# Gaius-Augustus/Augustus

Hardware: AMD Instinct MI355X
Metric: Mbp DNA decoded/sec (whole node), ab-initio human model (higher is better)
Workload: dtype f64; 1 GPU; synthetic uniform-random DNA, 100 contigs x 1000000 bp per GPU, --species=human ab initio (47 states, sample=0); pieces_in_flight_per_gpu=100, batches_in_flight_per_gpu=1

## Files before the change

augustus_amd/__init__.py:

```python
import ctypes
import sys
import os

_HERE = os.path.dirname(os.path.abspath(__file__))
LIB_PATH = os.environ.get("AUGX_LIB") or os.path.join(_HERE, "libaugx.so")

AUGX_E_ARG = -1
AUGX_E_NODEVICE = -3
AUGX_E_HIP = -4
AUGX_E_UNSUPPORTED = -5
AUGX_E_NOPATH = -6
AUGX_E_NOMEM = -7
AUGX_E_RANGE = -8


class AugxError(RuntimeError):
    def __init__(self, code, msg):
        super().__init__("augx error %d: %s" % (code, msg))
        self.code = code


class _Piece(ctypes.Structure):
    _fields_ = [("seq", ctypes.c_char_p), ("len", ctypes.c_int64), ("init_kind", ctypes.c_int32),
                ("term_kind", ctypes.c_int32)]
# ... 24 lines not shown
        L.augx_model_tables.restype = ctypes.c_void_p
        L.augx_model_tables.argtypes = [ctypes.c_void_p]
        L.augx_model_option.restype = ctypes.c_char_p
        L.augx_model_option.argtypes = [ctypes.c_void_p, ctypes.c_char_p]
        L.augx_model_destroy.argtypes = [ctypes.c_void_p]
        L.augx_device_count.restype = ctypes.c_int
        L.augx_partition_lpt.argtypes = [ctypes.c_void_p, ctypes.c_int, ctypes.c_int, ctypes.c_void_p]
        L.augx_decode_sharded.argtypes = [ctypes.c_void_p, ctypes.c_int, ctypes.c_void_p, ctypes.c_int, ctypes.c_void_p]
        L.augx_decoder_create.argtypes = [ctypes.c_void_p, ctypes.c_int, ctypes.POINTER(ctypes.c_void_p)]
        L.augx_decoder_destroy.argtypes = [ctypes.c_void_p]
        L.augx_decoder_set_share.argtypes = [ctypes.c_void_p, ctypes.c_int]
        L.augx_decoder_set_exact.argtypes = [ctypes.c_void_p, ctypes.c_int]
        L.augx_decoder_batch_capacity.restype = ctypes.c_int64
        L.augx_decoder_batch_capacity.argtypes = [ctypes.c_void_p]
        L.augx_batch_create.argtypes = [ctypes.c_void_p, ctypes.c_void_p, ctypes.c_int, ctypes.POINTER(ctypes.c_void_p)]
        L.augx_batch_decode.argtypes = [ctypes.c_void_p, ctypes.c_void_p]
        L.augx_batch_sync.argtypes = [ctypes.c_void_p]
        L.augx_batch_paths.argtypes = [ctypes.c_void_p, ctypes.c_void_p, ctypes.c_void_p]
        L.augx_batch_cells.argtypes = [ctypes.c_void_p, ctypes.c_void_p, ctypes.c_int, ctypes.c_void_p]
        L.augx_batch_prep.argtypes = [ctypes.c_void_p, ctypes.c_void_p, ctypes.c_int, ctypes.c_int, ctypes.c_int, ctypes.c_void_p, ctypes.c_int64,
                                      ctypes.POINTER(ctypes.c_int64)]
        L.augx_batch_kernel_ms.argtypes = [ctypes.c_void_p, ctypes.c_void_p, ctypes.POINTER(ctypes.c_float),
                                           ctypes.POINTER(ctypes.c_float), ctypes.POINTER(ctypes.c_float)]
        L.augx_batch_forward.argtypes = [ctypes.c_void_p, ctypes.c_void_p]
        L.augx_batch_forward_cells.argtypes = [ctypes.c_void_p, ctypes.c_void_p, ctypes.c_int, ctypes.c_void_p, ctypes.POINTER(ctypes.c_double)]
        L.augx_batch_destroy.argtypes = [ctypes.c_void_p]
        L.augx_rand_create.restype = ctypes.c_void_p
        L.augx_rand_create.argtypes = [ctypes.c_uint]
        L.augx_rand_next.argtypes = [ctypes.c_void_p]
        L.augx_rand_destroy.argtypes = [ctypes.c_void_p]
        L.augx_batch_sample.argtypes = [ctypes.c_void_p, ctypes.c_void_p, ctypes.c_int, ctypes.c_int, ctypes.c_void_p, ctypes.c_void_p]
        L.augx_decode_sampled.argtypes = [ctypes.c_void_p, ctypes.c_int, ctypes.c_void_p, ctypes.c_int, ctypes.c_int, ctypes.c_void_p,
                                          ctypes.c_void_p, ctypes.c_void_p]
        L.augx_format_gff_sampled.argtypes = [ctypes.c_void_p, ctypes.c_char_p, ctypes.c_char_p, ctypes.c_int64, ctypes.c_void_p, ctypes.c_int,
                                              ctypes.c_int, ctypes.c_void_p, ctypes.c_void_p, ctypes.c_int, ctypes.c_char_p, ctypes.c_int64,
                                              ctypes.POINTER(ctypes.c_int)]
        L.augx_path_free.argtypes = [ctypes.c_void_p]
        _lib = L
    return _lib


def _check(rc):
    if rc != 0:
        raise AugxError(rc, lib().augx_last_error().decode(errors="replace"))


# ... 65 lines not shown


class DecodedPiece:
    __slots__ = ("status", "ln_viterbi", "states")

    def __init__(self, status, lnv, states):
        self.status, self.ln_viterbi, self.states = status, lnv, states


class Batch:

    def __init__(self, decoder, seqs, init_kind=0, term_kind=0):
        L = lib()
        self.decoder = decoder
        self.n = len(seqs)
        self._keep = [s if isinstance(s, bytes) else s.encode() for s in seqs]
        self.lens = [len(s) for s in self._keep]
        P = (_Piece * self.n)()
        iks = init_kind if isinstance(init_kind, (list, tuple)) else [init_kind] * self.n
        tks = term_kind if isinstance(term_kind, (list, tuple)) else [term_kind] * self.n
        for i, s in enumerate(self._keep):
            P[i].seq, P[i].len, P[i].init_kind, P[i].term_kind = s, len(s), iks[i], tks[i]
        self._h = ctypes.c_void_p()
        _check(L.augx_batch_create(decoder._h, P, self.n, ctypes.byref(self._h)))
        decoder._batches.add(self._h.value)

    def decode(self, sync=True):
        _check(lib().augx_batch_decode(self.decoder._h, self._h))
        if sync:
            _check(lib().augx_batch_sync(self.decoder._h))

    def kernel_ms(self):
        a, b, c = ctypes.c_float(), ctypes.c_float(), ctypes.c_float()
        _check(lib().augx_batch_kernel_ms(self.decoder._h, self._h, ctypes.byref(a), ctypes.byref(b), ctypes.byref(c)))
        return {"prep_ms": a.value, "trellis_ms": b.value, "backtrace_ms": c.value}

    def paths(self):
        L = lib()
        out = (_Path * self.n)()
        _check(L.augx_batch_paths(self.decoder._h, self._h, out))
        res = []
        for i in range(self.n):
            st = [(out[i].states[k].begin, out[i].states[k].end, out[i].states[k].state, out[i].states[k].type)
                  for k in range(out[i].n_states)]
            res.append(DecodedPiece(out[i].status, out[i].ln_viterbi, st))
            L.augx_path_free(ctypes.byref(out[i]))
        return res

    def cells(self, piece):
        import numpy as np
        S = self.decoder.model.n_states
        V = np.empty((self.lens[piece], S), dtype=np.float64)
        _check(lib().augx_batch_cells(self.decoder._h, self._h, piece, V.ctypes.data_as(ctypes.c_void_p)))
        return V

    def prep(self, piece, which, plane=0):
        L = lib()
        return prep_fetch(lambda w, pl, out, cap, nb: L.augx_batch_prep(self.decoder._h, self._h, piece, w, pl, out, cap, nb), which, plane)

    def forward(self):
        _check(lib().augx_batch_forward(self.decoder._h, self._h))

    def forward_cells(self, piece):
        import numpy as np
        S = self.decoder.model.n_states
        F = np.empty((self.lens[piece], S), dtype=np.float64)
        lnp = ctypes.c_double()
        _check(lib().augx_batch_forward_cells(self.decoder._h, self._h, piece, F.ctypes.data_as(ctypes.c_void_p), ctypes.byref(lnp)))
        return F, lnp.value

    def sample(self, piece, n, rand):
        L = lib()
        out = (_Path * max(1, n))()
        _check(L.augx_batch_sample(self.decoder._h, self._h, piece, n, rand._h, out))
        res = []
        for i in range(n):
            if out[i].status != 0:
                raise AugxError(out[i].status, "sampling failed")
            res.append([(out[i].states[k].begin, out[i].states[k].end, out[i].states[k].state, out[i].states[k].type)
                        for k in range(out[i].n_states)])
            L.augx_path_free(ctypes.byref(out[i]))
# ... 83 lines not shown

def find_cuts(model, seqs, decode_fn, scout=-1):
    L = lib()
    L.augx_find_cuts.argtypes = [ctypes.c_void_p, ctypes.c_int, ctypes.POINTER(ctypes.c_char_p), ctypes.POINTER(ctypes.c_int64), DECODE_FN, ctypes.c_void_p,
                                 ctypes.c_int, ctypes.POINTER(ctypes.POINTER(_Cut)), ctypes.POINTER(ctypes.c_int), ctypes.POINTER(_CutStats)]
    L.augx_cuts_free.argtypes = [ctypes.POINTER(_Cut)]
    keep = [s.encode() if isinstance(s, str) else s for s in seqs]
    n = len(keep)
    c_seqs = (ctypes.c_char_p * n)(*keep)
    c_lens = (ctypes.c_int64 * n)(*[len(s) for s in keep])
    out = ctypes.POINTER(_Cut)()
    n_out = ctypes.c_int()
    st = _CutStats()
    _check(L.augx_find_cuts(model._h, n, c_seqs, c_lens, decode_fn, None, scout, ctypes.byref(out), ctypes.byref(n_out), ctypes.byref(st)))
    res = [(out[i].record, out[i].status, out[i].begin, out[i].end, out[i].init_kind, out[i].term_kind) for i in range(n_out.value)]
    L.augx_cuts_free(out)
    return res, {"scout_tiles": st.scout_tiles, "batches": st.batches, "windows_decoded": st.windows_decoded, "windows_used": st.windows_used}


def device_count():
    return lib().augx_device_count()


def partition_lpt(lens, n_bins):
    import numpy as np
    a = np.asarray(lens, dtype=np.int64)
    out = np.zeros(len(a), dtype=np.int32)
    _check(lib().augx_partition_lpt(a.ctypes.data_as(ctypes.c_void_p), len(a), n_bins, out.ctypes.data_as(ctypes.c_void_p)))
    return out.tolist()


def decode_sharded(decoders, seqs, init_kind=0, term_kind=0):
    L = lib()
    n = len(seqs)
    keep = [s if isinstance(s, bytes) else s.encode() for s in seqs]
    P = (_Piece * n)()
    iks = init_kind if isinstance(init_kind, (list, tuple)) else [init_kind] * n
    tks = term_kind if isinstance(term_kind, (list, tuple)) else [term_kind] * n
    for i, s in enumerate(keep):
        P[i].seq, P[i].len, P[i].init_kind, P[i].term_kind = s, len(s), iks[i], tks[i]
    D = (ctypes.c_void_p * len(decoders))(*[d._h for d in decoders])
    out = (_Path * n)()
    _check(L.augx_decode_sharded(D, len(decoders), P, n, out))
    res = []
    for i in range(n):
        st = [(out[i].states[k].begin, out[i].states[k].end, out[i].states[k].state, out[i].states[k].type)
# ... 54 lines not shown
```

augustus_amd/csrc/device/decoder.hip:

```cpp
#include <hip/hip_runtime.h>
#include <sys/mman.h>
#include <algorithm>
#include <map>
#include <array>
#include <cmath>
#include <unordered_map>
#include <cstdio>
#include <cstdlib>
#include <cstring>
#include <future>
#include <memory>
#include <mutex>
#include <set>
#include <string>
#include <system_error>
#include <thread>
#include <atomic>
#include <chrono>
#include <vector>
#include "kernels.h"
#include "dense.h"
#include "layout.h"
#include "launch.h"
#include "assmemo.h"
// ... 788 lines not shown
    keep(V.lnv, n); keep(V.status, n); keep(V.finalState, n); keep(V.pathCount, n);
    {
        std::vector<double> v;
        {
            std::lock_guard<std::mutex> lk(g_tss0Mu);
            if (!g_tss0Of.empty() && d->dense && d->hostT.utr)
                for (int p = 0; p < n; p++) {
                    auto it = g_tss0Of.find(pieces[p].seq);
                    if (it == g_tss0Of.end()) continue;
                    if (v.empty()) v.assign((size_t)n * 2, std::nan(""));
                    v[(size_t)p * 2] = it->second[0]; v[(size_t)p * 2 + 1] = it->second[1];
                }
        }
        if (!v.empty()) {
            double *dv = nullptr;
            keep(dv, (int64_t)n * 2);
            if (rc) return rc;
            if (hipMemcpy(dv, v.data(), sizeof(double) * v.size(), hipMemcpyHostToDevice) != hipSuccess) { setLastError("augx_batch_create: upload failed"); return AUGX_E_HIP; }
            V.tss0 = dv;
        }
    }
    keep(V.pathRec, Z.pathCap * 3);
    b->plan = planSegments(L, d->model->m.t, d->nCU / d->share > 0 ? d->nCU / d->share : 1, d->dense ? -1 : 0);
    SegDesc *dSegs = nullptr; int32_t *dSeg0 = nullptr;
    const int nSegs = (int)b->plan.segs.size();
    keep(dSegs, nSegs); keep(dSeg0, n + 1);
    V.nSegs = nSegs; V.segs = dSegs; V.pieceSeg0 = dSeg0; V.segCheckTiles = b->plan.checkTiles;
    if (const char *e = getenv("AUGX_SEG_CHECK_TILES")) V.segCheckTiles = atoi(e);
    keep(V.segStop, nSegs); keep(V.segStatus, nSegs); keep(V.segD, nSegs); keep(V.brkPos, nSegs); keep(V.brkOff, nSegs);
    keep(V.segStop2, nSegs); keep(V.segD2, nSegs); keep(V.pieceCovered, n);
    if (b->plan.cut()) {
        keep(V.ckRing, (int64_t)nSegs * 2 * WAVE * SP); keep(V.ckCol, Z.N / WAVE * SP);
        keep(V.tileMinEop, Z.N / WAVE); keep(V.tileCross, Z.N / WAVE);
    }
    keep(b->dV, 1);
    if (rc) return rc;
    const double tAlloc = getenv("AUGX_TIMING") ? std::chrono::duration<double>(std::chrono::steady_clock::now().time_since_epoch()).count() : 0.0;
    HIP_TRY(hipMemcpy(dOff, L.off.data(), sizeof(int64_t) * (n + 1), hipMemcpyHostToDevice));
    HIP_TRY(hipMemcpy(dLen, L.len.data(), sizeof(int32_t) * n, hipMemcpyHostToDevice));
    HIP_TRY(hipMemcpy(dIk, L.initKind.data(), sizeof(int32_t) * n, hipMemcpyHostToDevice));
    HIP_TRY(hipMemcpy(dTk, L.termKind.data(), sizeof(int32_t) * n, hipMemcpyHostToDevice));
    HIP_TRY(hipMemcpy(dCp, L.chunkPiece.data(), sizeof(int32_t) * L.nChunks, hipMemcpyHostToDevice));
    HIP_TRY(hipMemcpy(dSegs, b->plan.segs.data(), sizeof(SegDesc) * nSegs, hipMemcpyHostToDevice));
    HIP_TRY(hipMemcpy(dSeg0, b->plan.pieceSeg0.data(), sizeof(int32_t) * (n + 1), hipMemcpyHostToDevice));
    HIP_TRY(hipMemset(dRaw, 'n', (size_t)Z.N));
    HIP_TRY(hipMemset(V.gcPlane, 0, (size_t)Z.N));
    for (int p = 0; p < n; p++)
        HIP_TRY(hipMemcpy(dRaw + L.off[p] + 1, pieces[p].seq, (size_t)L.len[p], hipMemcpyHostToDevice));
    HIP_TRY(hipMemcpy(b->dV, &V, sizeof(BatchView), hipMemcpyHostToDevice));
    for (auto &e : b->ev) HIP_TRY(hipEventCreate(&e));
    if (tAlloc > 0) fprintf(stderr, "augx timing:       batch created: uploads + events %.3f s after the allocations (hipMalloc calls of this decoder so far: %.3f s for %.1f GB)\n",
                            std::chrono::duration<double>(std::chrono::steady_clock::now().time_since_epoch()).count() - tAlloc, d->mallocSeconds, d->mallocBytes / 1e9);
    *out = b.release();
    return AUGX_OK;
}

int augx_batch_decode(augx_decoder *d, augx_batch *b) {
    if (!d || !b) { setLastError("augx_batch_decode: NULL argument"); return AUGX_E_ARG; }
    HIP_TRY(hipSetDevice(d->device));
    const BatchView &V = b->V;
    const int n = V.nPieces;
    const unsigned gridN = (unsigned)((V.N + 255) / 256);
    hipStream_t st = d->stream;
    HIP_TRY(hipEventRecord(b->ev[0], st));
    b->memoReplayed = false;
    b->memoOf.clear();
    hipLaunchKernelGGL(kEncode, dim3(gridN), dim3(256), 0, st, V);
// ... 144 lines not shown
            }
            HIP_TRY(hipMemcpyAsync(b->dV, &W, sizeof(BatchView), hipMemcpyHostToDevice, st));
        }
    }
    if (timingFirst) {
        tf[4] = nowS();
        fprintf(stderr, "augx timing:       first decode of the batch, host side: class kernels + stairs %.3f s, stairs on the host + list sizes %.3f s, per-class / list arrays (%d planes) %.3f s, "
                        "prep launches + candidate buffer + candidates counted %.3f s (hipMalloc so far: %.3f s for %.1f GB)\n", tf[1] - tf[0], tf[2] - tf[1], b->V.nPl, tf[3] - tf[2], tf[4] - tf[3],
                d->mallocSeconds, d->mallocBytes / 1e9);
    }
    if (b->plan.cut()) hipLaunchKernelGGL(kTileCross, dim3((unsigned)((V.N / WAVE + 255) / 256)), dim3(256), 0, st, V);
    HIP_TRY(hipEventRecord(b->ev[1], st));
    auto runTrellis = [&]() -> int {
    if (d->dense) {
        launchDense(d->blk, 0, V.nearTie, (unsigned)n, st, d->dT, b->dV);
        HIP_TRY(hipGetLastError());
        HIP_TRY(hipEventRecord(b->ev[2], st));
        hipLaunchKernelGGL(kDenseBacktrace, dim3(n), dim3(64), 0, st, d->dT, V);
        HIP_TRY(hipGetLastError());
        return AUGX_OK;
    }
    HIP_TRY(hipMemsetAsync(V.segStatus, 0, sizeof(int32_t) * V.nSegs, st));
#define AUGX_LAUNCH_TRELLIS(MODE_, grid_) launchTrellis(d->blk, MODE_, V.nearTie, (unsigned)(grid_), st, d->dT, b->dV)
    AUGX_LAUNCH_TRELLIS(0, V.nSegs);
    if (b->plan.cut()) {
        HIP_TRY(hipMemsetAsync(V.segStop2, 0xFF, sizeof(int32_t) * V.nSegs, st));
        HIP_TRY(hipMemsetAsync(V.pieceCovered, 0xFF, sizeof(int32_t) * n, st));
        AUGX_LAUNCH_TRELLIS(1, V.nSegs);
        for (int round = 0; round < SEG_CONT_ROUNDS; round++) AUGX_LAUNCH_TRELLIS(2, n);
        AUGX_LAUNCH_TRELLIS(3, n);
    }
#undef AUGX_LAUNCH_TRELLIS
    hipLaunchKernelGGL(kSegFinalize, dim3((n + 63) / 64), dim3(64), 0, st, V);
    HIP_TRY(hipGetLastError());
    HIP_TRY(hipEventRecord(b->ev[2], st));
    hipLaunchKernelGGL(kBacktrace, dim3(n), dim3(64), 0, st, d->dT, V);
    HIP_TRY(hipGetLastError());
    return AUGX_OK;
    };
    int rcT = runTrellis();
    if (rcT) return rcT;
    b->decoded = true;
    if (d->exactMulti && b->nPlAlloc > 1) {
        int64_t nPatched = 0;
        int rc2;
        const bool timing = getenv("AUGX_TIMING") != nullptr;
        auto now = [] { return std::chrono::duration<double>(std::chrono::steady_clock::now().time_since_epoch()).count(); };
        if (timing) (void)hipStreamSynchronize(st);
        const double t0 = timing ? now() : 0.0;
        bool sitesRebuilt = false;
        try {
            rc2 = d->dense ? snippetCacheReplay(d, b, nPatched, false, b->V.cells) : snippetCacheReplay(d, b, nPatched, true, nullptr);
            if (!rc2 && d->dense && d->hostT.utr) rc2 = utrCachesReplay(d, b, b->V.cells, sitesRebuilt);
        } catch (const std::exception &e) { setLastError(std::string("augx_batch_decode: replay of the reference's caches: ") + e.what()); return AUGX_E_NOMEM; }
        if (rc2) return rc2;
        const double t1 = timing ? now() : 0.0;
        if ((nPatched > 0 || sitesRebuilt) && (rc2 = runTrellis())) return rc2;
        if (timing) {
            (void)hipStreamSynchronize(st);
            fprintf(stderr, "augx timing:     pieces with several GC classes: snippet-cache replay %.3f s (%lld candidate terms rebuilt), second trellis run %.3f s\n", t1 - t0, (long long)nPatched, now() - t1);
        }
    }
    HIP_TRY(hipEventRecord(b->ev[3], st));
    return AUGX_OK;
}

int augx_batch_sync(augx_decoder *d) {
    if (!d) return AUGX_E_ARG;
    HIP_TRY(hipSetDevice(d->device));
    HIP_TRY(hipStreamSynchronize(d->stream));
    return AUGX_OK;
}

int augx_batch_kernel_ms(augx_decoder *d, augx_batch *b, float *prep_ms, float *trellis_ms, float *back_ms) {
    if (!d || !b || !b->decoded) return AUGX_E_ARG;
    HIP_TRY(hipSetDevice(d->device));
    HIP_TRY(hipEventSynchronize(b->ev[3]));
    float a = 0, c = 0, e = 0;
    HIP_TRY(hipEventElapsedTime(&a, b->ev[0], b->ev[1]));
    HIP_TRY(hipEventElapsedTime(&c, b->ev[1], b->ev[2]));
    HIP_TRY(hipEventElapsedTime(&e, b->ev[2], b->ev[3]));
    if (prep_ms) *prep_ms = a;
    if (trellis_ms) *trellis_ms = c;
    if (back_ms) *back_ms = e;
    if (b->V.prof && d->dense) {
        std::vector<uint64_t> h((size_t)b->L.nPieces * 56 + 64);
// ... 860 lines not shown
```

augustus_amd/csrc/device/dp.h:

```cpp
#pragma once
#include <stdint.h>
#include <math.h>
#include "../../../include/augx.h"

#ifdef AUGX_EMU
#define AUGX_HD inline
#else
#include <hip/hip_runtime.h>
#define AUGX_HD __host__ __device__ __forceinline__
#endif

#if defined(__HIP_DEVICE_COMPILE__)
#define AUGX_GTAB(p) (p)
#else
#define AUGX_GTAB(p) (p)
#endif

namespace augx {
namespace dev {

constexpr int WAVE = 64;
constexpr int SP = 48;
constexpr int SPX = AUGX_MAX_STATES;
constexpr int NUFX = 6;
// ... 141 lines not shown
    double *longV;
    int32_t *laPos; double *laVal;
    int32_t *lrPos; double *lrVal;
    struct IntronStart *ldEnt; double *ldVal;
    struct IntronStart *rdEnt; double *rdVal;
    int32_t *atgPos;
    double *laPls; uint64_t *laFx;
    double *lrEt; uint64_t *lrFx;
    double *atgD; uint64_t *atgFx;
    int32_t *rsPos; double *rsBegin; uint64_t *rsFx;
    double *plsR;
    int blk;
    int64_t nBlk;
    uint32_t *blkCnt;
    uint32_t *blkSplit;
    uint64_t *blkOff;
    struct CandAlloc *candAlloc;
    Item *items;
    int64_t itemCap;
    int nSegs;
    const SegDesc *segs;
    const int32_t *pieceSeg0;
    int segCheckTiles;
    int32_t *tileMinEop;
    int32_t *tileCross;
    double *ckRing;
    double *ckCol;
    int32_t *segStop;
    double *segD;
    int32_t *segStop2;
    double *segD2;
    int32_t *pieceCovered;
    int32_t *segStatus;
    int32_t *brkPos;
    double *brkOff;
    double *lnv;
    int32_t *status;
    int32_t *finalState;
    int32_t *pathRec;
    int32_t *pathCount;
};

AUGX_HD int mod3(int k) { return k >= 0 ? k % 3 : (k % 3 + 3) % 3; }
AUGX_HD bool isUtrIntronKind(int k) { return k == AUGX_K_UTR5INTRON || k == AUGX_K_UTR3INTRON || k == AUGX_K_RUTR5INTRON || k == AUGX_K_RUTR3INTRON; }
AUGX_HD bool isUtrIntronVarKind(int k) { return k == AUGX_K_UTR5INTRONVAR || k == AUGX_K_UTR3INTRONVAR || k == AUGX_K_RUTR5INTRONVAR || k == AUGX_K_RUTR3INTRONVAR; }
AUGX_HD bool isUtrExonKind(int k) { return k >= AUGX_K_UTR5SINGLE && k <= AUGX_K_RUTR3TERM && !isUtrIntronKind(k) && !isUtrIntronVarKind(k); }
// ... 429 lines not shown
```

augustus_amd/csrc/device/k_trellis.hip:

```cpp
#include "kernels.h"
#include "launch.h"

using namespace augx;
using namespace augx::dev;

template <int BLK, int MODE, bool TIES> __global__ void __launch_bounds__(NT) kTrellis(const DevTables *__restrict__ T, const BatchView *__restrict__ B) {
    __shared__ TrellisLds lds;
    if constexpr (!TIES) {
        const int w = __builtin_amdgcn_readfirstlane((int)(threadIdx.x >> 6));
        switch (w) {
            case 0: trellisPiece<BLK, MODE, TIES, 0>(*T, *B, lds, blockIdx.x); break;
            case 1: trellisPiece<BLK, MODE, TIES, 1>(*T, *B, lds, blockIdx.x); break;
            case 2: trellisPiece<BLK, MODE, TIES, 2>(*T, *B, lds, blockIdx.x); break;
            case 3: trellisPiece<BLK, MODE, TIES, 3>(*T, *B, lds, blockIdx.x); break;
            case 4: trellisPiece<BLK, MODE, TIES, 4>(*T, *B, lds, blockIdx.x); break;
            case 5: trellisPiece<BLK, MODE, TIES, 5>(*T, *B, lds, blockIdx.x); break;
            case 6: trellisPiece<BLK, MODE, TIES, 6>(*T, *B, lds, blockIdx.x); break;
            default: trellisPiece<BLK, MODE, TIES, 7>(*T, *B, lds, blockIdx.x); break;
        }
    } else
        trellisPiece<BLK, MODE, TIES>(*T, *B, lds, blockIdx.x);
}

namespace augx { namespace dev {
void AUGX_TU_NAME(launchTrellis_)(int mode, bool ties, unsigned grid, hipStream_t st, const DevTables *T, const BatchView *B) {
    constexpr int BLK = AUGX_TU_BLK;
#define L(MODE_) do { if (ties) hipLaunchKernelGGL((kTrellis<BLK, MODE_, true>), dim3(grid), dim3(NT), 0, st, T, B); \
                      else hipLaunchKernelGGL((kTrellis<BLK, MODE_, false>), dim3(grid), dim3(NT), 0, st, T, B); } while (0)
    switch (mode) { case 0: L(0); break; case 1: L(1); break; case 2: L(2); break; default: L(3); break; }
#undef L
}
}}
```

augustus_amd/csrc/device/launch.h:

```cpp
#pragma once
#include <hip/hip_runtime.h>
#include "dp.h"

namespace augx { namespace dev {
void launchTrellis(int blk, int mode, bool ties, unsigned grid, hipStream_t st, const DevTables *T, const BatchView *B);
void launchCand(int blk, bool multi, bool dense, unsigned grid, hipStream_t st, const DevTables *T, const BatchView &W);
void launchForward(int blk, unsigned grid, hipStream_t st, const DevTables *T, const BatchView *B);
void launchDense(int blk, int mode, bool ties, unsigned grid, hipStream_t st, const DevTables *T, const BatchView *B);
void launchUtrDesc(int blk, unsigned grid, hipStream_t st, const DevTables *T, const BatchView &W);

#define AUGX_DECL_TU(BLK_)                                                                                                     \
    void launchTrellis_##BLK_(int mode, bool ties, unsigned grid, hipStream_t st, const DevTables *T, const BatchView *B);     \
    void launchCand_##BLK_(bool multi, bool dense, unsigned grid, hipStream_t st, const DevTables *T, const BatchView &W);     \
    void launchForward_##BLK_(unsigned grid, hipStream_t st, const DevTables *T, const BatchView *B);                          \
    void launchDense_##BLK_(int mode, bool ties, unsigned grid, hipStream_t st, const DevTables *T, const BatchView *B);       \
    void launchUtrDesc_##BLK_(unsigned grid, hipStream_t st, const DevTables *T, const BatchView &W);
AUGX_DECL_TU(8) AUGX_DECL_TU(4) AUGX_DECL_TU(2)
#undef AUGX_DECL_TU
#define AUGX_TU_CAT2(a, b) a##b
#define AUGX_TU_CAT(a, b) AUGX_TU_CAT2(a, b)
#define AUGX_TU_NAME(f) AUGX_TU_CAT(f, AUGX_TU_BLK)
}}
```

augustus_amd/csrc/device/layout.h:

```cpp
#pragma once
#include <cstdlib>
#include <cstring>
#include <stdexcept>
#include <string>
#include <vector>
#include "dp.h"

namespace augx {
namespace dev {

struct BatchLayout {
    int nPieces = 0;
    int64_t N = 0;
    int nChunks = 0;
    std::vector<int64_t> off;
    std::vector<int32_t> len, initKind, termKind, chunkPiece;
    void build(const augx_piece *pieces, int n) {
        nPieces = n;
        off.assign(n + 1, 0);
        len.resize(n); initKind.resize(n); termKind.resize(n);
        for (int p = 0; p < n; p++) {
            if (pieces[p].len < 1 || pieces[p].len >= 2900000) throw std::runtime_error("augx: piece length out of range (device pieces are shorter than 2.9 Mbp; lower --maxDNAPieceSize)");
            len[p] = (int32_t)pieces[p].len;
            initKind[p] = pieces[p].init_kind;
// ... 41 lines not shown
    for (int k = 0; k < R; k++) {
        int &m = map[cl[k]];
        if (m < 0) {
            if (nPl >= MAXPL) return -1;
            planeCls[nPl] = cl[k];
            m = nPl++;
        }
        const int e = k + 1 < R ? st[k + 1] : n;
        memset(plane.data() + st[k], m, (size_t)(e - st[k]));
    }
    return nPl;
}

inline int64_t listOffsets(const int32_t *listCnt, int nPieces, std::vector<int64_t> &offs) {
    offs.assign((size_t)nPieces + 1, 0);
    for (int p = 0; p < nPieces; p++) offs[p + 1] = offs[p] + (((int64_t)listCnt[p] + 1 + 63) / 64) * 64;
    return offs[nPieces] + 64;
}

constexpr int SEG_CONT_ROUNDS = 3;
struct SegPlan {
    std::vector<SegDesc> segs;
    std::vector<int32_t> pieceSeg0;
    int checkTiles = 0;
    bool cut() const { return segs.size() + 1 > pieceSeg0.size(); }
};
inline int segCheckTiles(const augx_tables &t) {
    int reach = t.max_exon_len > t.d ? t.max_exon_len : t.d;
    reach += t.W + t.U + 64;
    return (reach + WAVE - 1) / WAVE + 4;
}
inline bool segmentsSupported(const augx_tables &t) {
    const int dL = t.d - 2 - t.De - t.As - 2 - t.U;
    return t.state_kind[t.synch_state] == AUGX_K_IGENIC && dL >= 4 * WAVE && t.reachable[t.synch_state];
}
inline SegPlan planSegments(const BatchLayout &L, const augx_tables &t, int slots, int segTiles = 0) {
    SegPlan P;
    P.checkTiles = segCheckTiles(t);
    const int n = L.nPieces;
    if (const char *e = getenv("AUGX_SEG_LEN")) { const long v = atol(e); segTiles = v <= 0 ? -1 : (int)((v + WAVE - 1) / WAVE); }
    const int minSeg = 5 * P.checkTiles;
    std::vector<int> tiles(n);
    int64_t total = 0;
    int maxTiles = 0;
    for (int p = 0; p < n; p++) { tiles[p] = (L.len[p] + WAVE - 1) / WAVE; total += tiles[p]; if (tiles[p] > maxTiles) maxTiles = tiles[p]; }
    if (!segmentsSupported(t)) segTiles = -1;
    auto countFor = [&](int st, int p) {
        int k = (tiles[p] + st / 2) / st;
        while (k > 1 && tiles[p] / k < minSeg) k--;
        return k < 1 ? 1 : k;
    };
    if (segTiles == 0) {
        const int64_t fixLen = 450;
        int64_t bestCost = -1;
        int best = -1;
        for (int k = 1; k <= 64; k++) {
            int st = (maxTiles + k - 1) / k;
            if (k > 1 && st < minSeg) break;
            int64_t nSeg = 0, nFix = 0, longest = 0;
            for (int p = 0; p < n; p++) {
                const int kp = k == 1 ? 1 : countFor(st, p);
                nSeg += kp; nFix += kp - 1;
                const int64_t len = (tiles[p] + kp - 1) / kp;
                if (len > longest) longest = len;
            }
            int64_t cost = (nSeg + slots - 1) / slots * longest + (nFix + slots - 1) / slots * fixLen;
            if (k > 1) cost += cost / 6;
            if (bestCost < 0 || cost < bestCost) { bestCost = cost; best = k == 1 ? -1 : st; }
        }
        segTiles = best;
    }
    if (segTiles > 0 && segTiles < minSeg) segTiles = minSeg;
    std::vector<int> kOf(n, 1);
    if (segTiles > 0) {
        int64_t nSeg = 0;
        for (int p = 0; p < n; p++) { kOf[p] = countFor(segTiles, p); nSeg += kOf[p]; }
        int extra = nSeg > slots ? (int)((slots - nSeg % slots) % slots) : 0;
        if (extra > 0 && extra <= n / 4 + 1)
            for (int p = 0; p < n && extra > 0; p++)
                if (kOf[p] > 1 && tiles[p] / (kOf[p] + 1) >= minSeg) { kOf[p]++; extra--; }
    }
    P.pieceSeg0.assign((size_t)n + 1, 0);
    for (int p = 0; p < n; p++) {
        const int kp = kOf[p];
        P.pieceSeg0[p] = (int32_t)P.segs.size();
        for (int k = 0; k < kp; k++) {
            SegDesc d;
            d.piece = p; d.k = k;
            d.t0 = (int32_t)((int64_t)tiles[p] * k / kp);
            d.t1 = (int32_t)((int64_t)tiles[p] * (k + 1) / kp);
            d.tlim = d.t1 - P.checkTiles - 2;
            d.pad = 0;
            P.segs.push_back(d);
        }
    }
    P.pieceSeg0[n] = (int32_t)P.segs.size();
    return P;
}

struct BatchSizes {
    int64_t N, nChunks, nPieces, pathCap;
    explicit BatchSizes(const BatchLayout &L) {
        N = L.N; nChunks = L.nChunks; nPieces = L.nPieces;
        pathCap = N / 8 + 64 * (int64_t)L.nPieces + 64;
    }
};

inline long long forwardCellCandidates(const augx_tables &t) {
    int len = t.max_exon_len > t.d ? t.max_exon_len : t.d;
    if (t.utr_max_exon_len > len) len = t.utr_max_exon_len;
    if (t.utr_max3single > len) len = t.utr_max3single;
    if (t.utr_max3term > len) len = t.utr_max3term;
    return (long long)AUGX_MAX_ANC * ((long long)len + 1);
}
static_assert((long long)AUGX_MAX_ANC * (0x3FFF + 1) <= FWD_SUM_TERMS, "the lengths 14-bit back pointers admit fit the forward sum");
inline void checkForwardSum(const augx_tables &t) {
    if (forwardCellCandidates(t) > FWD_SUM_TERMS) throw std::runtime_error("augx: exon or intron lengths too large for the fixed-point sums of the forward pass");
// ... 232 lines not shown
```

include/augx.h:

```cpp
#ifndef AUGX_H
#define AUGX_H
#include <stdint.h>
#ifdef __cplusplus
extern "C" {
#endif

#define AUGX_MAX_STATES 80
#define AUGX_MAX_ANC 8
#define AUGX_MAX_CLASSES 16
#define AUGX_Q_BITS 31
#define AUGX_FX_SHIFT 40
#define AUGX_FX_SCALE 1099511627776.0
#define AUGX_FX_INV (1.0 / 1099511627776.0)

enum {
    AUGX_OK = 0,
    AUGX_E_ARG = -1,
    AUGX_E_CONFIG = -2,
    AUGX_E_NODEVICE = -3,
    AUGX_E_HIP = -4,
    AUGX_E_UNSUPPORTED = -5,
    AUGX_E_NOPATH = -6,
    AUGX_E_NOMEM = -7,
    AUGX_E_RANGE = -8
// ... 144 lines not shown
int augx_tss0(const augx_model *m, const char *seq, int64_t len, double *out );
int augx_tss0_override(const char *seq, const double *v );
int augx_decode_sharded(augx_decoder *const *decs, int n_dec, const augx_piece *pieces, int n, augx_path *out );

typedef int (*augx_decode_fn)(void *user, const augx_piece *pieces, int n, augx_path *out );
typedef struct augx_cut {
    int32_t record;
    int32_t status;
    int64_t begin, end;
    int32_t init_kind, term_kind;
} augx_cut;
typedef struct augx_cut_stats { int32_t scout_tiles, batches, windows_decoded, windows_used; } augx_cut_stats;
int augx_find_cuts(const augx_model *m, int n_records, const char *const *seqs, const int64_t *lens, augx_decode_fn fn, void *user,
                   int scout , augx_cut **out, int *n_out,
                   augx_cut_stats *stats );
void augx_cuts_free(augx_cut *c);

typedef struct augx_batch augx_batch;
int augx_batch_create(augx_decoder *d, const augx_piece *pieces, int n, augx_batch **out);
int augx_batch_decode(augx_decoder *d, augx_batch *b);
int augx_batch_sync(augx_decoder *d);
int augx_batch_paths(augx_decoder *d, augx_batch *b, augx_path *out );
int augx_batch_kernel_ms(augx_decoder *d, augx_batch *b, float *prep_ms, float *trellis_ms, float *back_ms);
int augx_batch_cells(augx_decoder *d, augx_batch *b, int piece, double *out);
enum { AUGX_PREP_CODE = 0, AUGX_PREP_CNT, AUGX_PREP_NSM, AUGX_PREP_GCRAW, AUGX_PREP_GCPLANE, AUGX_PREP_FX, AUGX_PREP_SIG, AUGX_PREP_GATE,
       AUGX_PREP_PLSR, AUGX_PREP_UFX, AUGX_PREP_UCNT, AUGX_PREP_CLS, AUGX_PREP_NPLANES, AUGX_PREP_PLANECLS, AUGX_PREP_LISTCNT, AUGX_PREP_N };
int augx_batch_prep(augx_decoder *d, augx_batch *b, int piece, int which, int plane, void *out, int64_t cap_bytes, int64_t *n_bytes);
int augx_batch_forward(augx_decoder *d, augx_batch *b);
int augx_batch_forward_cells(augx_decoder *d, augx_batch *b, int piece, double *out, double *ln_p);
typedef struct augx_rand augx_rand;
augx_rand *augx_rand_create(unsigned seed);
int augx_rand_next(augx_rand *r);
void augx_rand_skip(augx_rand *r, int64_t n);
void augx_rand_destroy(augx_rand *r);
int augx_batch_sample(augx_decoder *d, augx_batch *b, int piece, int n_samples, augx_rand *r, augx_path *out );
int augx_decode_sampled(augx_decoder *const *decs, int n_dec, const augx_piece *pieces, int n, int n_samples, augx_rand *r,
                        augx_path *out , augx_path *samples );
void augx_batch_destroy(augx_batch *b);

int augx_main(int argc, const char *const *argv);

int augx_format_gff(const augx_model *m, const char *name, const char *seq, int64_t len, const augx_state *states,
                    int n_states, int first_gene_id, char *out, int64_t out_cap, int *n_genes);
int augx_format_gff_sampled(const augx_model *m, const char *name, const char *seq, int64_t len, const augx_state *states,
                            int n_states, int n_samples, const augx_state *const *sample_states, const int *sample_n,
                            int first_gene_id, char *out, int64_t out_cap, int *n_genes);
// ... 19 lines not shown
```

Before: 490.3 Mbp/s.

## Pack trellis segments into balanced per-block runs via binary-searched bin packing

Adds a run-based segment plan: pieces are laid end to end and cut so that each workgroup processes a contiguous run of segments whose total tile length is bounded by a binary-searched limit. The trellis kernel gains a RUNS variant that loops over the segments of its run. The planner picks this over the per-piece uniform split when its estimated cost is lower, and the fix-up cost model is refined. The aim is fewer idle compute units and fewer cut fix-ups. The cost is more planner complexity and extra block syncs between segments, and a wrong cut could hurt when runs straddle pieces. New plan-query APIs and a timing printout are added as well.

```diff
diff --git a/augustus_amd/__init__.py b/augustus_amd/__init__.py
--- a/augustus_amd/__init__.py
+++ b/augustus_amd/__init__.py
@@ -70,6 +70,10 @@
                                       ctypes.POINTER(ctypes.c_int64)]
         L.augx_batch_kernel_ms.argtypes = [ctypes.c_void_p, ctypes.c_void_p, ctypes.POINTER(ctypes.c_float),
                                            ctypes.POINTER(ctypes.c_float), ctypes.POINTER(ctypes.c_float)]
+        _plan = [ctypes.c_void_p, ctypes.c_int, ctypes.POINTER(ctypes.c_int), ctypes.c_void_p, ctypes.c_int, ctypes.POINTER(ctypes.c_int),
+                 ctypes.POINTER(ctypes.c_int), ctypes.c_void_p]
+        L.augx_plan_segments.argtypes = [ctypes.c_void_p, ctypes.c_void_p, ctypes.c_int, ctypes.c_int] + _plan
+        L.augx_batch_plan.argtypes = [ctypes.c_void_p, ctypes.c_void_p] + _plan + [ctypes.c_void_p, ctypes.c_void_p]
         L.augx_batch_forward.argtypes = [ctypes.c_void_p, ctypes.c_void_p]
         L.augx_batch_forward_cells.argtypes = [ctypes.c_void_p, ctypes.c_void_p, ctypes.c_int, ctypes.c_void_p, ctypes.POINTER(ctypes.c_double)]
         L.augx_batch_destroy.argtypes = [ctypes.c_void_p]
@@ -181,11 +185,13 @@
         for i, s in enumerate(self._keep):
             P[i].seq, P[i].len, P[i].init_kind, P[i].term_kind = s, len(s), iks[i], tks[i]
         self._h = ctypes.c_void_p()
+        self._decoded = False
         _check(L.augx_batch_create(decoder._h, P, self.n, ctypes.byref(self._h)))
         decoder._batches.add(self._h.value)
 
     def decode(self, sync=True):
         _check(lib().augx_batch_decode(self.decoder._h, self._h))
+        self._decoded = True
         if sync:
             _check(lib().augx_batch_sync(self.decoder._h))
 
@@ -216,6 +222,12 @@
     def prep(self, piece, which, plane=0):
         L = lib()
         return prep_fetch(lambda w, pl, out, cap, nb: L.augx_batch_prep(self.decoder._h, self._h, piece, w, pl, out, cap, nb), which, plane)
+
+    def plan(self):
+        L = lib()
+        if not self._decoded:
+            return _plan_query(lambda *a: L.augx_batch_plan(self.decoder._h, self._h, *a, None, None))
+        return _plan_query(lambda *a: L.augx_batch_plan(self.decoder._h, self._h, *a), stops=True)
 
     def forward(self):
         _check(lib().augx_batch_forward(self.decoder._h, self._h))
@@ -345,6 +357,31 @@
     return lib().augx_device_count()
 
 
+def _plan_query(call, stops=False):
+    import numpy as np
+    ns, nr, ck = ctypes.c_int(), ctypes.c_int(), ctypes.c_int()
+    est = np.zeros(2, dtype=np.int64)
+    _check(call(None, 0, ctypes.byref(ns), None, 0, ctypes.byref(nr), ctypes.byref(ck), est.ctypes.data_as(ctypes.c_void_p), *((None, None) if stops else ())))
+    segs = np.zeros((ns.value, 5), dtype=np.int32)
+    runs = np.zeros(nr.value + 1, dtype=np.int32)
+    more = ()
+    if stops:
+        more = (np.full(ns.value, -1, dtype=np.int32), np.full(ns.value, -1, dtype=np.int32))
+    _check(call(segs.ctypes.data_as(ctypes.c_void_p), ns.value, ctypes.byref(ns), runs.ctypes.data_as(ctypes.c_void_p), nr.value, ctypes.byref(nr),
+                ctypes.byref(ck), est.ctypes.data_as(ctypes.c_void_p), *[None if a is None else a.ctypes.data_as(ctypes.c_void_p) for a in more]))
+    res = {"segs": segs, "run_seg0": runs[:nr.value + 1] if nr.value else runs[:0], "n_runs": nr.value, "check_tiles": ck.value,
+           "est_tiles": int(est[0]), "est_per_piece": int(est[1])}
+    res["seg_stop"], res["seg_stop2"] = more if stops else (None, None)
+    return res
+
+
+def plan_segments(model, lens, slots):
+    import numpy as np
+    a = np.ascontiguousarray(lens, dtype=np.int64)
+    L = lib()
+    return _plan_query(lambda *args: L.augx_plan_segments(model.tables_ptr, a.ctypes.data_as(ctypes.c_void_p), len(a), slots, *args))
+
+
 def partition_lpt(lens, n_bins):
     import numpy as np
     a = np.asarray(lens, dtype=np.int64)
diff --git a/augustus_amd/csrc/device/decoder.hip b/augustus_amd/csrc/device/decoder.hip
--- a/augustus_amd/csrc/device/decoder.hip
+++ b/augustus_amd/csrc/device/decoder.hip
@@ -834,10 +834,12 @@
     }
     keep(V.pathRec, Z.pathCap * 3);
     b->plan = planSegments(L, d->model->m.t, d->nCU / d->share > 0 ? d->nCU / d->share : 1, d->dense ? -1 : 0);
-    SegDesc *dSegs = nullptr; int32_t *dSeg0 = nullptr;
-    const int nSegs = (int)b->plan.segs.size();
+    SegDesc *dSegs = nullptr; int32_t *dSeg0 = nullptr, *dRun0 = nullptr;
+    const int nSegs = (int)b->plan.segs.size(), nRuns = b->plan.nRuns();
     keep(dSegs, nSegs); keep(dSeg0, n + 1);
+    if (nRuns > 0) keep(dRun0, nRuns + 1);
     V.nSegs = nSegs; V.segs = dSegs; V.pieceSeg0 = dSeg0; V.segCheckTiles = b->plan.checkTiles;
+    V.nRuns = nRuns; V.runSeg0 = dRun0;
     if (const char *e = getenv("AUGX_SEG_CHECK_TILES")) V.segCheckTiles = atoi(e);
     keep(V.segStop, nSegs); keep(V.segStatus, nSegs); keep(V.segD, nSegs); keep(V.brkPos, nSegs); keep(V.brkOff, nSegs);
     keep(V.segStop2, nSegs); keep(V.segD2, nSegs); keep(V.pieceCovered, n);
@@ -855,6 +857,7 @@
     HIP_TRY(hipMemcpy(dCp, L.chunkPiece.data(), sizeof(int32_t) * L.nChunks, hipMemcpyHostToDevice));
     HIP_TRY(hipMemcpy(dSegs, b->plan.segs.data(), sizeof(SegDesc) * nSegs, hipMemcpyHostToDevice));
     HIP_TRY(hipMemcpy(dSeg0, b->plan.pieceSeg0.data(), sizeof(int32_t) * (n + 1), hipMemcpyHostToDevice));
+    if (nRuns > 0) HIP_TRY(hipMemcpy(dRun0, b->plan.runSeg0.data(), sizeof(int32_t) * (nRuns + 1), hipMemcpyHostToDevice));
     HIP_TRY(hipMemset(dRaw, 'n', (size_t)Z.N));
     HIP_TRY(hipMemset(V.gcPlane, 0, (size_t)Z.N));
     for (int p = 0; p < n; p++)
@@ -1045,7 +1048,8 @@
     }
     HIP_TRY(hipMemsetAsync(V.segStatus, 0, sizeof(int32_t) * V.nSegs, st));
 #define AUGX_LAUNCH_TRELLIS(MODE_, grid_) launchTrellis(d->blk, MODE_, V.nearTie, (unsigned)(grid_), st, d->dT, b->dV)
-    AUGX_LAUNCH_TRELLIS(0, V.nSegs);
+    if (V.nRuns > 0) AUGX_LAUNCH_TRELLIS(TRELLIS_RUNS, V.nRuns);
+    else AUGX_LAUNCH_TRELLIS(0, V.nSegs);
     if (b->plan.cut()) {
         HIP_TRY(hipMemsetAsync(V.segStop2, 0xFF, sizeof(int32_t) * V.nSegs, st));
         HIP_TRY(hipMemsetAsync(V.pieceCovered, 0xFF, sizeof(int32_t) * n, st));
@@ -1085,6 +1089,75 @@
         }
     }
     HIP_TRY(hipEventRecord(b->ev[3], st));
+    if (timingFirst && !d->dense) {
+        const SegPlan &P = b->plan;
+        int longestSeg = 0, longestRun = 0, gaveUp = 0;
+        for (const SegDesc &sd : P.segs) if (sd.t1 - sd.t0 > longestSeg) longestSeg = sd.t1 - sd.t0;
+        for (int r = 0; r < P.nRuns(); r++) {
+            int len = 0;
+            for (int q = P.runSeg0[r]; q < P.runSeg0[r + 1]; q++) len += P.segs[q].t1 - P.segs[q].t0;
+            if (len > longestRun) longestRun = len;
+        }
+        if (P.cut()) {
+            std::vector<int32_t> stop(P.segs.size());
+            HIP_TRY(hipStreamSynchronize(st));
+            HIP_TRY(hipMemcpy(stop.data(), V.segStop, sizeof(int32_t) * stop.size(), hipMemcpyDeviceToHost));
+            for (size_t q = 0; q < stop.size(); q++) gaveUp += P.segs[q].k > 0 && stop[q] <= -2;
+        }
+        fprintf(stderr, "augx timing:       trellis plan: %d segments of %d pieces, %d runs, longest run %d tiles, longest segment %d tiles, estimate %lld tiles (pieces cut one by one: %lld); %d fix-ups gave up\n",
+                (int)P.segs.size(), n, P.nRuns(), longestRun, longestSeg, (long long)P.estTiles, (long long)P.estPerPiece, gaveUp);
+    }
+    return AUGX_OK;
+}
+
+namespace {
+int planOut(const SegPlan &P, int32_t *segs, int cap_segs, int *n_segs, int32_t *run_seg0, int cap_runs, int *n_runs, int *check_tiles, int64_t *est) {
+    const int nS = (int)P.segs.size(), nR = P.nRuns();
+    if (n_segs) *n_segs = nS;
+    if (n_runs) *n_runs = nR;
+    if (check_tiles) *check_tiles = P.checkTiles;
+    if (est) { est[0] = P.estTiles; est[1] = P.estPerPiece; }
+    if ((segs && cap_segs < nS) || (run_seg0 && cap_runs < nR)) { setLastError("augx plan query: output arrays too small"); return AUGX_E_ARG; }
+    if (segs)
+        for (int q = 0; q < nS; q++) {
+            const SegDesc &sd = P.segs[q];
+            int32_t *o = segs + (size_t)q * 5;
+            o[0] = sd.piece; o[1] = sd.k; o[2] = sd.t0; o[3] = sd.t1; o[4] = sd.tlim;
+        }
+    if (run_seg0)
+        for (int r = 0; r <= nR && nR > 0; r++) run_seg0[r] = P.runSeg0[r];
+    return AUGX_OK;
+}
+}
+
+int augx_plan_segments(const augx_tables *t, const int64_t *lens, int n, int slots, int32_t *segs, int cap_segs, int *n_segs,
+                       int32_t *run_seg0, int cap_runs, int *n_runs, int *check_tiles, int64_t *est) {
+    if (!t || !lens || n < 1 || slots < 1) { setLastError("augx_plan_segments: bad argument"); return AUGX_E_ARG; }
+    try {
+        std::vector<augx_piece> pieces((size_t)n);
+        for (int p = 0; p < n; p++) { pieces[p].seq = nullptr; pieces[p].len = lens[p]; pieces[p].init_kind = 0; pieces[p].term_kind = 0; }
+        BatchLayout L;
+        L.build(pieces.data(), n);
+        return planOut(planSegments(L, *t, slots, modelIsDense(*t) ? -1 : 0), segs, cap_segs, n_segs, run_seg0, cap_runs, n_runs, check_tiles, est);
+    } catch (const std::exception &e) { setLastError(std::string("augx_plan_segments: ") + e.what()); return AUGX_E_ARG; }
+}
+
+int augx_batch_plan(augx_decoder *d, augx_batch *b, int32_t *segs, int cap_segs, int *n_segs, int32_t *run_seg0, int cap_runs, int *n_runs,
+                    int *check_tiles, int64_t *est, int32_t *seg_stop, int32_t *seg_stop2) {
+    if (!d || !b) { setLastError("augx_batch_plan: NULL argument"); return AUGX_E_ARG; }
+    const int rc = planOut(b->plan, segs, cap_segs, n_segs, run_seg0, cap_runs, n_runs, check_tiles, est);
+    if (rc || (!seg_stop && !seg_stop2)) return rc;
+    const size_t nS = b->plan.segs.size();
+    if (cap_segs < (int)nS) { setLastError("augx_batch_plan: output arrays too small"); return AUGX_E_ARG; }
+    if (!b->decoded) { setLastError("augx_batch_plan: the batch has not been decoded"); return AUGX_E_ARG; }
+    if (!b->plan.cut()) {
+        for (size_t q = 0; q < nS; q++) { if (seg_stop) seg_stop[q] = -1; if (seg_stop2) seg_stop2[q] = -1; }
+        return AUGX_OK;
+    }
+    HIP_TRY(hipSetDevice(d->device));
+    HIP_TRY(hipStreamSynchronize(d->stream));
+    if (seg_stop) HIP_TRY(hipMemcpy(seg_stop, b->V.segStop, sizeof(int32_t) * nS, hipMemcpyDeviceToHost));
+    if (seg_stop2) HIP_TRY(hipMemcpy(seg_stop2, b->V.segStop2, sizeof(int32_t) * nS, hipMemcpyDeviceToHost));
     return AUGX_OK;
 }
 
diff --git a/augustus_amd/csrc/device/dp.h b/augustus_amd/csrc/device/dp.h
--- a/augustus_amd/csrc/device/dp.h
+++ b/augustus_amd/csrc/device/dp.h
@@ -187,6 +187,8 @@
     const SegDesc *segs;
     const int32_t *pieceSeg0;
     int segCheckTiles;
+    int nRuns;
+    const int32_t *runSeg0;
     int32_t *tileMinEop;
     int32_t *tileCross;
     double *ckRing;
diff --git a/augustus_amd/csrc/device/k_trellis.hip b/augustus_amd/csrc/device/k_trellis.hip
--- a/augustus_amd/csrc/device/k_trellis.hip
+++ b/augustus_amd/csrc/device/k_trellis.hip
@@ -4,22 +4,32 @@
 using namespace augx;
 using namespace augx::dev;
 
-template <int BLK, int MODE, bool TIES> __global__ void __launch_bounds__(NT) kTrellis(const DevTables *__restrict__ T, const BatchView *__restrict__ B) {
+template <int BLK, int MODE, bool TIES, bool RUNS = false> __global__ void __launch_bounds__(NT) kTrellis(const DevTables *__restrict__ T, const BatchView *__restrict__ B) {
+    static_assert(!RUNS || MODE == 0, "runs are pass 1");
     __shared__ TrellisLds lds;
-    if constexpr (!TIES) {
-        const int w = __builtin_amdgcn_readfirstlane((int)(threadIdx.x >> 6));
-        switch (w) {
-            case 0: trellisPiece<BLK, MODE, TIES, 0>(*T, *B, lds, blockIdx.x); break;
-            case 1: trellisPiece<BLK, MODE, TIES, 1>(*T, *B, lds, blockIdx.x); break;
-            case 2: trellisPiece<BLK, MODE, TIES, 2>(*T, *B, lds, blockIdx.x); break;
-            case 3: trellisPiece<BLK, MODE, TIES, 3>(*T, *B, lds, blockIdx.x); break;
-            case 4: trellisPiece<BLK, MODE, TIES, 4>(*T, *B, lds, blockIdx.x); break;
-            case 5: trellisPiece<BLK, MODE, TIES, 5>(*T, *B, lds, blockIdx.x); break;
-            case 6: trellisPiece<BLK, MODE, TIES, 6>(*T, *B, lds, blockIdx.x); break;
-            default: trellisPiece<BLK, MODE, TIES, 7>(*T, *B, lds, blockIdx.x); break;
-        }
-    } else
-        trellisPiece<BLK, MODE, TIES>(*T, *B, lds, blockIdx.x);
+    int sg = blockIdx.x, sgEnd = sg + 1;
+    if constexpr (RUNS) {
+        sg = __builtin_amdgcn_readfirstlane(B->runSeg0[blockIdx.x]);
+        sgEnd = __builtin_amdgcn_readfirstlane(B->runSeg0[blockIdx.x + 1]);
+    }
+    for (;;) {
+        if constexpr (!TIES) {
+            const int w = __builtin_amdgcn_readfirstlane((int)(threadIdx.x >> 6));
+            switch (w) {
+                case 0: trellisPiece<BLK, MODE, TIES, 0>(*T, *B, lds, sg); break;
+                case 1: trellisPiece<BLK, MODE, TIES, 1>(*T, *B, lds, sg); break;
+                case 2: trellisPiece<BLK, MODE, TIES, 2>(*T, *B, lds, sg); break;
+                case 3: trellisPiece<BLK, MODE, TIES, 3>(*T, *B, lds, sg); break;
+                case 4: trellisPiece<BLK, MODE, TIES, 4>(*T, *B, lds, sg); break;
+                case 5: trellisPiece<BLK, MODE, TIES, 5>(*T, *B, lds, sg); break;
+                case 6: trellisPiece<BLK, MODE, TIES, 6>(*T, *B, lds, sg); break;
+                default: trellisPiece<BLK, MODE, TIES, 7>(*T, *B, lds, sg); break;
+            }
+        } else
+            trellisPiece<BLK, MODE, TIES>(*T, *B, lds, sg);
+        if (!RUNS || ++sg >= sgEnd) break;
+        BLOCK_SYNC();
+    }
 }
 
 namespace augx { namespace dev {
@@ -27,6 +37,11 @@
     constexpr int BLK = AUGX_TU_BLK;
 #define L(MODE_) do { if (ties) hipLaunchKernelGGL((kTrellis<BLK, MODE_, true>), dim3(grid), dim3(NT), 0, st, T, B); \
                       else hipLaunchKernelGGL((kTrellis<BLK, MODE_, false>), dim3(grid), dim3(NT), 0, st, T, B); } while (0)
+    if (mode == TRELLIS_RUNS) {
+        if (ties) hipLaunchKernelGGL((kTrellis<BLK, 0, true, true>), dim3(grid), dim3(NT), 0, st, T, B);
+        else hipLaunchKernelGGL((kTrellis<BLK, 0, false, true>), dim3(grid), dim3(NT), 0, st, T, B);
+        return;
+    }
     switch (mode) { case 0: L(0); break; case 1: L(1); break; case 2: L(2); break; default: L(3); break; }
 #undef L
 }
diff --git a/augustus_amd/csrc/device/launch.h b/augustus_amd/csrc/device/launch.h
--- a/augustus_amd/csrc/device/launch.h
+++ b/augustus_amd/csrc/device/launch.h
@@ -3,6 +3,7 @@
 #include "dp.h"
 
 namespace augx { namespace dev {
+constexpr int TRELLIS_RUNS = 4;
 void launchTrellis(int blk, int mode, bool ties, unsigned grid, hipStream_t st, const DevTables *T, const BatchView *B);
 void launchCand(int blk, bool multi, bool dense, unsigned grid, hipStream_t st, const DevTables *T, const BatchView &W);
 void launchForward(int blk, unsigned grid, hipStream_t st, const DevTables *T, const BatchView *B);
diff --git a/augustus_amd/csrc/device/layout.h b/augustus_amd/csrc/device/layout.h
--- a/augustus_amd/csrc/device/layout.h
+++ b/augustus_amd/csrc/device/layout.h
@@ -87,8 +87,12 @@
 struct SegPlan {
     std::vector<SegDesc> segs;
     std::vector<int32_t> pieceSeg0;
+    std::vector<int32_t> runSeg0;
     int checkTiles = 0;
+    int64_t estTiles = 0;
+    int64_t estPerPiece = 0;
     bool cut() const { return segs.size() + 1 > pieceSeg0.size(); }
+    int nRuns() const { return runSeg0.empty() ? 0 : (int)runSeg0.size() - 1; }
 };
 inline int segCheckTiles(const augx_tables &t) {
     int reach = t.max_exon_len > t.d ? t.max_exon_len : t.d;
@@ -98,6 +102,65 @@
 inline bool segmentsSupported(const augx_tables &t) {
     const int dL = t.d - 2 - t.De - t.As - 2 - t.U;
     return t.state_kind[t.synch_state] == AUGX_K_IGENIC && dL >= 4 * WAVE && t.reachable[t.synch_state];
+}
+constexpr int64_t SEG_FIX_MEAN = 374, SEG_FIX_PER_BIT = 100, SEG_FIX_ROUND = 570;
+inline int64_t segFixTiles(int64_t nFix, int slots) {
+    if (nFix <= 0) return 0;
+    const int64_t rounds = (nFix + slots - 1) / slots, first = nFix < slots ? nFix : slots;
+    int bits = 0;
+    while ((first >> bits) > 0) bits++;
+    return SEG_FIX_MEAN + SEG_FIX_PER_BIT * bits + (rounds - 1) * SEG_FIX_ROUND;
+}
+struct RunCuts {
+    std::vector<std::pair<int, int>> cuts;
+    std::vector<std::pair<int, int>> runStart;
+    int64_t longest = 0;
+};
+inline bool cutRunsWithin(const std::vector<int> &tiles, int64_t B, int slots, int minSeg, int headMin, RunCuts *out) {
+    const int n = (int)tiles.size();
+    auto tileable = [&](int64_t rmin) -> int64_t {
+        if (B < minSeg) return -1;
+        if (rmin < minSeg) rmin = minSeg;
+        const int64_t m = (rmin + B - 1) / B;
+        return m * minSeg <= rmin ? rmin : m * minSeg;
+    };
+    if (out) { out->cuts.clear(); out->runStart.clear(); out->longest = 0; }
+    int p = 0, c = 0, runs = 0;
+    while (p < n) {
+        if (++runs > slots) return false;
+        if (out) out->runStart.push_back({p, c});
+        int64_t used = 0;
+        const int64_t rem = tiles[p] - c;
+        if (rem > B) {
+            const int64_t r = tileable(rem - B), low = c == 0 ? headMin : minSeg;
+            if (r < 0 || rem - r < low) return false;
+            c = (int)(tiles[p] - r); used = rem - r;
+            if (out) out->cuts.push_back({p, c});
+        } else {
+            used = rem; p++; c = 0;
+            while (p < n && used + tiles[p] <= B) used += tiles[p++];
+            if (p < n) {
+                const int64_t r = tileable(tiles[p] - (B - used));
+                if (r >= 0 && tiles[p] - r >= headMin) {
+                    c = (int)(tiles[p] - r); used += c;
+                    if (out) out->cuts.push_back({p, c});
+                }
+            }
+        }
+        if (out && used > out->longest) out->longest = used;
+    }
+    return true;
+}
+inline bool planRuns(const std::vector<int> &tiles, int slots, int minSeg, int headMin, RunCuts &R) {
+    int64_t total = 0;
+    for (int t : tiles) total += t;
+    if (total <= 0 || slots < 1) return false;
+    int64_t lo = (total + slots - 1) / slots - 1, hi = total;
+    while (hi - lo > 1) {
+        const int64_t mid = lo + (hi - lo) / 2;
+        if (cutRunsWithin(tiles, mid, slots, minSeg, headMin, nullptr)) hi = mid; else lo = mid;
+    }
+    return cutRunsWithin(tiles, hi, slots, minSeg, headMin, &R);
 }
 inline SegPlan planSegments(const BatchLayout &L, const augx_tables &t, int slots, int segTiles = 0) {
     SegPlan P;
@@ -105,6 +168,7 @@
     const int n = L.nPieces;
     if (const char *e = getenv("AUGX_SEG_LEN")) { const long v = atol(e); segTiles = v <= 0 ? -1 : (int)((v + WAVE - 1) / WAVE); }
     const int minSeg = 5 * P.checkTiles;
+    const int headMin = P.checkTiles + 2;
     std::vector<int> tiles(n);
     int64_t total = 0;
     int maxTiles = 0;
@@ -115,8 +179,9 @@
         while (k > 1 && tiles[p] / k < minSeg) k--;
         return k < 1 ? 1 : k;
     };
+    RunCuts R;
+    bool useRuns = false;
     if (segTiles == 0) {
-        const int64_t fixLen = 450;
         int64_t bestCost = -1;
         int best = -1;
         for (int k = 1; k <= 64; k++) {
@@ -129,11 +194,43 @@
                 const int64_t len = (tiles[p] + kp - 1) / kp;
                 if (len > longest) longest = len;
             }
-            int64_t cost = (nSeg + slots - 1) / slots * longest + (nFix + slots - 1) / slots * fixLen;
-            if (k > 1) cost += cost / 6;
-            if (bestCost < 0 || cost < bestCost) { bestCost = cost; best = k == 1 ? -1 : st; }
+            int64_t cost = (nSeg + slots - 1) / slots * longest + segFixTiles(nFix, slots);
+            if (nFix > 0) cost += cost / 6;
+            if (bestCost < 0 || cost < bestCost) { bestCost = cost; best = nFix == 0 ? -1 : st; }
         }
         segTiles = best;
+        P.estPerPiece = P.estTiles = bestCost;
+        if (n > 0 && planRuns(tiles, slots, minSeg, headMin, R) && !R.cuts.empty()) {
+            int64_t cost = R.longest + segFixTiles((int64_t)R.cuts.size(), slots);
+            cost += cost / 6;
+            if (cost < bestCost) { useRuns = true; P.estTiles = cost; }
+        }
+    }
+    P.pieceSeg0.assign((size_t)n + 1, 0);
+    auto addSeg = [&](int p, int k, int t0, int t1) {
+        SegDesc d;
+        d.piece = p; d.k = k; d.t0 = t0; d.t1 = t1;
+        d.tlim = d.t1 - P.checkTiles - 2;
+        d.pad = 0;
+        P.segs.push_back(d);
+    };
+    if (useRuns) {
+        size_t ci = 0, ri = 0;
+        for (int p = 0; p < n; p++) {
+            P.pieceSeg0[p] = (int32_t)P.segs.size();
+            int k = 0, t0 = 0;
+            for (;; k++) {
+                if (ri < R.runStart.size() && R.runStart[ri].first == p && R.runStart[ri].second == t0) { P.runSeg0.push_back((int32_t)P.segs.size()); ri++; }
+                const bool more = ci < R.cuts.size() && R.cuts[ci].first == p;
+                const int t1 = more ? R.cuts[ci].second : tiles[p];
+                addSeg(p, k, t0, t1);
+                if (!more) break;
+                t0 = t1; ci++;
+            }
+        }
+        P.pieceSeg0[n] = (int32_t)P.segs.size();
+        P.runSeg0.push_back((int32_t)P.segs.size());
+        return P;
     }
     if (segTiles > 0 && segTiles < minSeg) segTiles = minSeg;
     std::vector<int> kOf(n, 1);
@@ -145,19 +242,11 @@
             for (int p = 0; p < n && extra > 0; p++)
                 if (kOf[p] > 1 && tiles[p] / (kOf[p] + 1) >= minSeg) { kOf[p]++; extra--; }
     }
-    P.pieceSeg0.assign((size_t)n + 1, 0);
     for (int p = 0; p < n; p++) {
         const int kp = kOf[p];
         P.pieceSeg0[p] = (int32_t)P.segs.size();
-        for (int k = 0; k < kp; k++) {
-            SegDesc d;
-            d.piece = p; d.k = k;
-            d.t0 = (int32_t)((int64_t)tiles[p] * k / kp);
-            d.t1 = (int32_t)((int64_t)tiles[p] * (k + 1) / kp);
-            d.tlim = d.t1 - P.checkTiles - 2;
-            d.pad = 0;
-            P.segs.push_back(d);
-        }
+        for (int k = 0; k < kp; k++)
+            addSeg(p, k, (int32_t)((int64_t)tiles[p] * k / kp), (int32_t)((int64_t)tiles[p] * (k + 1) / kp));
     }
     P.pieceSeg0[n] = (int32_t)P.segs.size();
     return P;
diff --git a/include/augx.h b/include/augx.h
--- a/include/augx.h
+++ b/include/augx.h
@@ -190,6 +190,10 @@
 int augx_batch_sync(augx_decoder *d);
 int augx_batch_paths(augx_decoder *d, augx_batch *b, augx_path *out );
 int augx_batch_kernel_ms(augx_decoder *d, augx_batch *b, float *prep_ms, float *trellis_ms, float *back_ms);
+int augx_plan_segments(const augx_tables *t, const int64_t *lens, int n, int slots, int32_t *segs , int cap_segs, int *n_segs,
+                       int32_t *run_seg0 , int cap_runs, int *n_runs, int *check_tiles, int64_t *est );
+int augx_batch_plan(augx_decoder *d, augx_batch *b, int32_t *segs, int cap_segs, int *n_segs, int32_t *run_seg0, int cap_runs, int *n_runs,
+                    int *check_tiles, int64_t *est, int32_t *seg_stop , int32_t *seg_stop2 );
 int augx_batch_cells(augx_decoder *d, augx_batch *b, int piece, double *out);
 enum { AUGX_PREP_CODE = 0, AUGX_PREP_CNT, AUGX_PREP_NSM, AUGX_PREP_GCRAW, AUGX_PREP_GCPLANE, AUGX_PREP_FX, AUGX_PREP_SIG, AUGX_PREP_GATE,
        AUGX_PREP_PLSR, AUGX_PREP_UFX, AUGX_PREP_UCNT, AUGX_PREP_CLS, AUGX_PREP_NPLANES, AUGX_PREP_PLANECLS, AUGX_PREP_LISTCNT, AUGX_PREP_N };
```

New measurement: 513.6 Mbp/s, median of 6. +4.7%, better.
